# zyddnys/manga-image-translator

Hardware: AMD Instinct MI355X
Metric: pages/sec end-to-end (detect+OCR+inpaint), 2048x1456 (higher is better)
Workload: dtype f32

## Files before the change

### include/mit_hip.h

```cpp
#ifndef MIT_HIP_H
#define MIT_HIP_H

#include <stdint.h>

#ifdef __cplusplus
extern "C" {
#endif

#define MIT_ABI_VERSION 23
#define MIT_MAX_TAPS 64

enum MitAct {
    MIT_ACT_NONE = 0,
    MIT_ACT_RELU = 1,
    MIT_ACT_LEAKY = 2,
    MIT_ACT_SILU = 3,
    MIT_ACT_SIGMOID = 4,
    MIT_ACT_GELU = 5
};
#define MIT_ACT_POST_FIRST 0x100

enum MitPad {
    MIT_PAD_ZERO = 0,
    MIT_PAD_REFLECT = 1
};

typedef struct MitTensorMap {
    float *base;
    int64_t zs1, zs0, bs, ys, xs;
    int64_t nhi;
    int32_t nsplit;
    int32_t _pad;
} MitTensorMap;

typedef struct MitConvGemm {
    const float *a;
    int64_t a_zs1, a_zs0, a_bs, a_ys, a_xs;
    int32_t NB, Hi, Wi, Cin;
    int32_t Ho, Wo, sy, sx;
    int32_t ntaps, pad_mode;
    int8_t tap_dy[MIT_MAX_TAPS];
    int8_t tap_dx[MIT_MAX_TAPS];
    int32_t tap_off[MIT_MAX_TAPS];
    const float *w;
    int64_t w_zs1, w_zs0, ldw;
    int32_t Kw, Nw;
    int32_t N;
    int32_t Z, zdiv;
    MitTensorMap c, pre, post;
    const float *scale, *bias;
    int32_t act;
    float act_alpha;
    const uint16_t *w_split;
    int64_t ws_zs0;
    const int32_t *lut_rows;
    const float *lut1, *lut2;
    int64_t lut_ld;
    int32_t nprod;
    int32_t live_img0;
    const int32_t *live_blocks;
    const int32_t *live_start;
    const float *wino_m;
// ... 1 lines not shown
    int32_t wino_n, wino_th, wino_tw;
    int32_t _pad_wino;
} MitConvGemm;

const char *mit_last_error(void);
int mit_abi_version(void);
const char *mit_source_digest(void);

int mit_device_count(int *count);
int mit_device_name(int device, char *buf, int buflen);

int mit_conv_gemm(const MitConvGemm *desc, void *stream);
int mit_conv_gemm_cfg(const MitConvGemm *desc, int cfg, void *stream);
const char *mit_conv_gemm_config_name(int cfg);
int mit_conv_gemm_plan(const MitConvGemm *desc, int cfg, int32_t *tile, int32_t *nb_run);
const char *mit_conv_gemm_config_kernel(int cfg);

int mit_gemm_split_pack(const float *w_dev, int64_t w_zs, int nz, int Kw, int64_t ldw, uint16_t *out_dev, void *stream);
int mit_gemm_mode_set(int mode);
int mit_gemm_mode_get(void);
int64_t mit_gemm_split_min_tiles(int64_t n);

typedef struct MitPGemm {
    const uint16_t *a_planes;
    int64_t a_zs;
    int64_t lda;
    const uint16_t *w_planes;
    int64_t w_zs;
    int64_t ldw;
    int32_t M, N, K, Z;
    float *c;
    int64_t ldc, c_zs;
    const float *pre;
    int64_t ld_pre, pre_zs;
    const float *post;
    int64_t ld_post, post_zs;
    uint16_t *c_planes;
    int64_t ld_cp, cp_zs;
    const float *scale, *bias;
    int32_t act;
    float act_alpha;
    int32_t nprod;
    int32_t tile;
} MitPGemm;
int mit_pgemm(const MitPGemm *desc, void *stream);
const char *mit_pgemm_tile_name(int tile);
int mit_pgemm_supported(const MitPGemm *desc);
int mit_split_planes(const float *x_dev, int64_t ldx, int R, int K, uint16_t *planes_dev, int64_t ld, void *stream);
int mit_join_planes(const uint16_t *planes_dev, int64_t ld, int R, int K, float *x_dev, int64_t ldx, void *stream);

int mit_conv_small_cout(const float *in_dev, int64_t in_pixstride, int64_t in_planestride, const float *w4_dev, const float *w_pairs_dev, const float *bias_dev, float *out_dev,
                        int64_t out_pixstride, int B, int H, int W, int Cin, int Cout, int k, int pad_mode, int act,
                        float act_alpha, const uint8_t *live_cells, void *stream);

int64_t mit_lama_tail_need_work(int B, int H, int W);
int mit_lama_tail_need(const uint8_t *mask_dev, int B, int H, int W, uint8_t *cells_dev, int32_t *list0_dev, int32_t *start0_dev, int32_t *list1_dev,
                       int32_t *start1_dev, int32_t *list2_dev, int32_t *start2_dev, uint8_t *work_dev, void *stream);

int mit_convnext_mlp_supported(int C);
int mit_convnext_mlp(const float *x_dev, int64_t ldx, int M, int C, const uint16_t *w1_planes_dev, const float *b1_dev,
                     const uint16_t *w2perm_planes_dev, int64_t ldn2, const float *scale2_dev, const float *bias2_dev,
                     const float *post_dev, int64_t ldp, float *out_dev, int64_t ldo, void *stream);

int mit_wino43_input(const float *x_dev, int64_t x_bs, int64_t x_ys, int64_t x_xs, float *v_dev, int B, int H, int W, int C,
                     int pad_mode, void *stream);
int mit_wino43_output(const float *m_dev, float *y_dev, int64_t y_bs, int64_t y_ys, int64_t y_xs, const float *post_dev,
                      int64_t p_bs, int64_t p_ys, int64_t p_xs, const float *scale_dev, const float *bias_dev, int B, int H,
                      int W, int N, int act, float alpha, void *stream);

typedef struct MitProfStat {
    int64_t launches;
    double ms, exec_flops, alg_flops;
} MitProfStat;
int mit_prof_enable(int on);
int mit_prof_tag_next(double alg_flops);
int mit_prof_read(MitProfStat *stats, int max_cfgs, int *n_cfgs);
int mit_prof_dump(const char *path);
typedef struct MitProfKernelStat {
    char name[48];
    int64_t launches;
    double ms, alg_bytes, alg_flops;
} MitProfKernelStat;
int mit_prof_kernels_read(MitProfKernelStat *stats, int max_stats, int *n_stats);

int mit_resize_u8(const uint8_t *src_dev, int B, int H, int W, int C, uint8_t *dst_dev, int dh, int dw, int mode, const int *yidx_dev,
                  const uint16_t *ycoef_dev, const int *xidx_dev, const uint16_t *xcoef_dev, void *stream);
int mit_resample_pil_u8(const uint8_t *src_dev, int B, int H, int W, int C, uint8_t *dst_dev, int n_out, int axis, const int *bounds_dev,
                        const int *coef_dev, int ksize, void *stream);
int mit_bilateral_u8c3(const uint8_t *src_dev, uint8_t *dst_dev, int B, int H, int W, int radius, int ntaps, const int *tap_ofs_dev,
                       const float *tap_w_dev, const float *color_w_dev, void *stream);
int mit_select_u8(const uint8_t *mask_dev, int thr, const uint8_t *a_dev, const uint8_t *b_dev, uint8_t *out_dev, int64_t npix, int C,
                  void *stream);

typedef struct MitRefineWindow {
    int x1, y1, x2, y2;
} MitRefineWindow;
typedef struct MitRefineCand {
    int kind;
    int lo, hi;
    int invert;
} MitRefineCand;
int64_t mit_ctd_refine_workspace_bytes(const MitRefineWindow *windows, int n);
int mit_ctd_refine_hist(const uint8_t *page_dev, const uint8_t *pred_dev, int H, int W, const MitRefineWindow *windows, int n, int *hist_host,
                        void *workspace_dev, int64_t workspace_bytes, void *stream);
int mit_ctd_refine_scores(const uint8_t *page_dev, const uint8_t *pred_dev, int H, int W, const MitRefineWindow *windows, int n,
                          const MitRefineCand *cands_host, uint64_t *sums_host, void *workspace_dev, int64_t workspace_bytes, void *stream);
// ... 285 lines not shown
```

### manga_image_translator_amd/ctd.py

```python
from __future__ import annotations

import ctypes as C
import math
from typing import Dict, Optional, Tuple

import numpy as np
import torch

from . import lib as _lib
from . import ops
from .ops import ACT_LEAKY, ACT_NONE, ACT_RELU, ACT_SIGMOID, ACT_SILU, bn_params

INPUT_SIZE = 1024


def _fused_yolo_conv(sd, p, k, s, device):
    w = sd[p + ".conv.weight"].to(torch.float32)
    bw, bb, rm, rv = (sd[p + ".bn." + n].to(torch.float32) for n in ("weight", "bias", "running_mean", "running_var"))
    eps = 1e-3
    scale = bw.div(torch.sqrt(eps + rv))
    fw = (w.reshape(w.shape[0], -1) * scale[:, None]).reshape(w.shape)
    fb = bb - bw.mul(rm).div(torch.sqrt(rv + eps))
    return ops.Conv2d(fw, fb, stride=s, padding=(2 if k == 6 else k // 2), act=ACT_SILU, device=device)


def _head_conv(sd, p, k, device):
    return ops.Conv2d(sd[p + ".conv.weight"], None, padding=k // 2, bn=bn_params(sd, p + ".bn"), act=ACT_LEAKY, alpha=0.1,
                      device=device)


class _C3:

    def __init__(self, sd, p, c1, c2, n, mk, shortcut=True):
        self.c_ = c2 // 2
        self.c2 = c2
        self.cv1, self.cv2, self.cv3 = mk(p + ".cv1", 1), mk(p + ".cv2", 1), mk(p + ".cv3", 1)
        self.m = [(mk(f"{p}.m.{j}.cv1", 1), mk(f"{p}.m.{j}.cv2", 3)) for j in range(n)]
        self.shortcut = shortcut

    def __call__(self, eng, x, out, tag):
        B, H, W, _ = x.shape
        cat = eng._buf(f"{tag}.cat", B, H, W, 2 * self.c_)
        y = cat[..., :self.c_]
        self.cv2(x, out=cat[..., self.c_:])
        self.cv1(x, out=y)
        t = eng._buf(f"{tag}.t", B, H, W, self.c_)
        for a, b in self.m:
            a(y, out=t)
            b(t, out=y, post=y if self.shortcut else None)
        return self.cv3(cat, out=out)


class CtdEngine(ops.Engine):

    def __init__(self, yolo_sd: Dict[str, torch.Tensor], seg_sd: Dict[str, torch.Tensor], det_sd: Dict[str, torch.Tensor],
                 device="cuda"):
        super().__init__(device)
        dev = self.device
        ymk = lambda k_s: (lambda p, k: _fused_yolo_conv(yolo_sd, p, k, k_s, dev))
        y1 = lambda p, k: _fused_yolo_conv(yolo_sd, p, k, 1, dev)
        self.y0 = _fused_yolo_conv(yolo_sd, "model.0", 6, 2, dev)
        self.y1 = _fused_yolo_conv(yolo_sd, "model.1", 3, 2, dev)
        self.y2 = _C3(yolo_sd, "model.2", 64, 64, 1, y1)
        self.y3 = _fused_yolo_conv(yolo_sd, "model.3", 3, 2, dev)
        self.y4 = _C3(yolo_sd, "model.4", 128, 128, 2, y1)
        self.y5 = _fused_yolo_conv(yolo_sd, "model.5", 3, 2, dev)
        self.y6 = _C3(yolo_sd, "model.6", 256, 256, 3, y1)
        self.y7 = _fused_yolo_conv(yolo_sd, "model.7", 3, 2, dev)
        self.y8 = _C3(yolo_sd, "model.8", 512, 512, 1, y1)
        self.y9a = y1("model.9.cv1", 1)
        self.y9b = y1("model.9.cv2", 1)

        def up_c3(sd, p, cin, mid, cout):
            hk = lambda q, k: _head_conv(sd, q, k, dev)
            c3 = _C3(sd, p + ".conv.0", cin, mid, 1, hk)
            up = ops.ConvTranspose2d(sd[p + ".conv.1.weight"], None, stride=2, padding=1, bn=bn_params(sd, p + ".conv.2"),
                                     act=ACT_RELU, device=dev)
            return c3, up

        s = seg_sd
        self.down1 = _C3(s, "down_conv1.conv", 512, 512, 1, lambda q, k: _head_conv(s, q, k, dev))
        self.up0 = up_c3(s, "upconv0", 512, 512, 256)
        self.up2 = up_c3(s, "upconv2", 768, 512, 256)
        self.up3 = up_c3(s, "upconv3", 512, 512, 256)
        self.up4 = up_c3(s, "upconv4", 384, 256, 128)
        self.up5 = up_c3(s, "upconv5", 192, 128, 64)
        self.up6 = ops.ConvTranspose2d(s["upconv6.0.weight"], None, stride=2, padding=1, act=ACT_SIGMOID, device=dev)
        d = det_sd
        self.d_up3 = up_c3(d, "upconv3", 512, 512, 256)
        self.d_up4 = up_c3(d, "upconv4", 384, 256, 128)
        self.d_conv = ops.Conv2d(d["conv.0.weight"], d["conv.0.bias"], bn=bn_params(d, "conv.1"), act=ACT_RELU, device=dev)

        def branch(p, first_bias):
            c0 = ops.Conv2d(d[p + ".0.weight"], d[p + ".0.bias"] if first_bias else None, padding=1, bn=bn_params(d, p + ".1"),
                            act=ACT_RELU, device=dev)
            t1 = ops.ConvTranspose2d(d[p + ".3.weight"], d[p + ".3.bias"], stride=2, bn=bn_params(d, p + ".4"), act=ACT_RELU,
                                     device=dev)
            t2 = ops.ConvTranspose2d(d[p + ".6.weight"], d[p + ".6.bias"], stride=2, act=ACT_SIGMOID, device=dev)
            return c0, t1, t2

        self.br_binarize = branch("binarize", True)
        self.br_thresh = branch("thresh", False)
        self._prep_tabs: Dict[Tuple, dict] = {}

    @staticmethod
    def letterbox_geometry(H: int, W: int, S: int = INPUT_SIZE):
        r = min(S / H, S / W)
        nw, nh = int(round(W * r)), int(round(H * r))
        return nh, nw, S - nw, S - nh

    def _resize_tables(self, H, W, nh, nw):
# ... 45 lines not shown
        if (nh, nw) == (H, W):
            mode, tb = 0, None
        elif H == 2 * nh and W == 2 * nw:
            mode, tb = 1, None
        else:
            mode, tb = 2, self._resize_tables(H, W, nh, nw)
        _lib.check(lib.mit_ctd_prep(pages_u8.data_ptr(), B, H, W, nh, nw, S, mode,
                                    tb["yi"].data_ptr() if tb else None, tb["yc"].data_ptr() if tb else None,
                                    tb["xi"].data_ptr() if tb else None, tb["xc"].data_ptr() if tb else None,
                                    x.data_ptr(), st), "mit_ctd_prep")
        if taps is not None:
            taps["input"] = x.clone()
        a0 = self._buf("y0", B, 512, 512, 32)
        self.y0(x, out=a0)
        cat160 = self._buf("cat160", B, 256, 256, 192)
        f160 = cat160[..., :64]
        self.y1(a0, out=f160)
        a2 = self._buf("y2", B, 256, 256, 64)
        self.y2(self, f160, a2, "y2")
        cat80 = self._buf("cat80", B, 128, 128, 384)
        f80 = cat80[..., :128]
        self.y3(a2, out=f80)
        a4 = self._buf("y4", B, 128, 128, 128)
        self.y4(self, f80, a4, "y4")
        cat40 = self._buf("cat40", B, 64, 64, 512)
        f40 = cat40[..., :256]
        self.y5(a4, out=f40)
        a6 = self._buf("y6", B, 64, 64, 256)
        self.y6(self, f40, a6, "y6")
        cat20 = self._buf("cat20", B, 32, 32, 768)
        f20 = cat20[..., :512]
        self.y7(a6, out=f20)
        a8 = self._buf("y8", B, 32, 32, 512)
        self.y8(self, f20, a8, "y8")
        sp = self._buf("sppf", B, 32, 32, 1024)
        self.y9a(a8, out=sp[..., :256])
        for j in range(3):
            src, dst = sp[..., 256 * j:256 * (j + 1)], sp[..., 256 * (j + 1):256 * (j + 2)]
            _lib.check(lib.mit_maxpool_nhwc(src.data_ptr(), 1024, dst.data_ptr(), 1024, B, 32, 32, 256, 5, st), "mit_maxpool_nhwc")
        f3 = self._buf("f3", B, 32, 32, 512)
        self.y9b(sp, out=f3)
        if taps is not None:
            taps.update(f160=f160.clone(), f80=f80.clone(), f40=f40.clone(), f20=f20.clone(), f3=f3.clone())
        p16 = self._buf("p16", B, 16, 16, 512)
        _lib.check(lib.mit_avgpool2_nhwc(f3.data_ptr(), 512, p16.data_ptr(), 512, B, 16, 16, 512, st), "mit_avgpool2_nhwc")
        d10 = self._buf("d10", B, 16, 16, 512)
        self.down1(self, p16, d10, "down1")
        self._up(self.up0, d10, cat20[..., 512:], "up0")
        self._up(self.up2, cat20, cat40[..., 256:], "up2")
        self._up(self.up3, cat40, cat80[..., 128:], "up3")
        self._up(self.up4, cat80, cat160[..., 64:], "up4")
        u320 = self._buf("u320", B, 512, 512, 64)
        self._up(self.up5, cat160, u320, "up5")
        mask = self._buf("mask", B, S, S, 1)
        self.up6(u320, out=mask)
        dcat80 = self._buf("dcat80", B, 128, 128, 384)
        _lib.check(lib.mit_copy_channels(f80.data_ptr(), 384, dcat80.data_ptr(), 384, B * 128 * 128, 128, st), "mit_copy_channels")
        self._up(self.d_up3, cat40, dcat80[..., 128:], "dup3")
        dx = self._buf("dx", B, 256, 256, 128)
        self._up(self.d_up4, dcat80, dx, "dup4")
        dc = self._buf("dc", B, 256, 256, 64)
        self.d_conv(dx, out=dc)
        lines = self._buf("lines", B, 2, S, S)
        for plane, (c0, t1, t2) in ((0, self.br_binarize), (1, self.br_thresh)):
            b0 = self._buf("db0", B, 256, 256, 16)
            c0(dc, out=b0)
            b1 = self._buf("db1", B, 512, 512, 16)
            t1(b0, out=b1)
            t2(b1, out=lines[:, plane].unsqueeze(-1))
        mask_u8 = self._buf("mask_u8", B, S, S, dtype=torch.uint8)
        _lib.check(lib.mit_map_to_u8(mask.data_ptr(), mask_u8.data_ptr(), B * S * S, 0, 0.0, st), "mit_map_to_u8")
        if taps is not None:
            taps["mask_f32"] = mask.clone()
        self.last_mask_f32 = mask[..., 0]
        return mask_u8[:, :S - dh, :S - dw], lines[:, :, :S - dh, :S - dw], (dw, dh)

    def shrink_bitmap(self, lines: torch.Tensor, thr: float = 0.3) -> torch.Tensor:
        shrink = lines[:, 0].contiguous()
        out = torch.empty(shrink.shape, dtype=torch.uint8, device=self.device)
        _lib.check(_lib.load().mit_map_to_u8(shrink.data_ptr(), out.data_ptr(), shrink.numel(), 1, thr,
                                             C.c_void_p(ops.current_stream())), "mit_map_to_u8")
        return out

    @staticmethod
    def flops_per_page() -> float:
        def conv(cin, cout, k, hw):
            return 2.0 * cin * cout * k * k * hw

        def c3(c1, c2, n, hw):
            c_ = c2 // 2
            return conv(c1, c_, 1, hw) * 2 + conv(2 * c_, c2, 1, hw) + n * (conv(c_, c_, 1, hw) + conv(c_, c_, 3, hw))

        f = conv(3, 32, 6, 512 ** 2) + conv(32, 64, 3, 256 ** 2) + c3(64, 64, 1, 256 ** 2) + conv(64, 128, 3, 128 ** 2)
        f += c3(128, 128, 2, 128 ** 2) + conv(128, 256, 3, 64 ** 2) + c3(256, 256, 3, 64 ** 2) + conv(256, 512, 3, 32 ** 2)
        f += c3(512, 512, 1, 32 ** 2) + conv(512, 256, 1, 32 ** 2) + conv(1024, 512, 1, 32 ** 2)

        def up(cin, mid, cout, hw):
            return c3(cin, mid, 1, hw) + conv(mid, cout, 4, hw)

        f += c3(512, 512, 1, 16 ** 2) + up(512, 512, 256, 16 ** 2) + up(768, 512, 256, 32 ** 2) + up(512, 512, 256, 64 ** 2)
        f += up(384, 256, 128, 128 ** 2) + up(192, 128, 64, 256 ** 2) + conv(64, 1, 4, 512 ** 2)
        f += up(512, 512, 256, 64 ** 2) + up(384, 256, 128, 128 ** 2) + conv(128, 64, 1, 256 ** 2)
        f += 2 * (conv(64, 16, 3, 256 ** 2) + conv(16, 16, 2, 256 ** 2) + conv(16, 1, 2, 512 ** 2))
        return f
```

### manga_image_translator_amd/lib.py

```python
from __future__ import annotations

import ctypes as C
from pathlib import Path

MIT_MAX_TAPS = 64
MIT_ABI_VERSION = 23

ACT_NONE, ACT_RELU, ACT_LEAKY, ACT_SILU, ACT_SIGMOID, ACT_GELU = range(6)
ACT_POST_FIRST = 0x100
PAD_ZERO, PAD_REFLECT = 0, 1


class MitTensorMap(C.Structure):
    _fields_ = [
        ("base", C.c_void_p),
        ("zs1", C.c_int64),
        ("zs0", C.c_int64),
        ("bs", C.c_int64),
        ("ys", C.c_int64),
        ("xs", C.c_int64),
        ("nhi", C.c_int64),
        ("nsplit", C.c_int32),
        ("_pad", C.c_int32),
    ]


class MitConvGemm(C.Structure):
    _fields_ = [
        ("a", C.c_void_p),
        ("a_zs1", C.c_int64),
        ("a_zs0", C.c_int64),
        ("a_bs", C.c_int64),
        ("a_ys", C.c_int64),
        ("a_xs", C.c_int64),
        ("NB", C.c_int32),
        ("Hi", C.c_int32),
        ("Wi", C.c_int32),
        ("Cin", C.c_int32),
        ("Ho", C.c_int32),
        ("Wo", C.c_int32),
        ("sy", C.c_int32),
        ("sx", C.c_int32),
        ("ntaps", C.c_int32),
        ("pad_mode", C.c_int32),
        ("tap_dy", C.c_int8 * MIT_MAX_TAPS),
        ("tap_dx", C.c_int8 * MIT_MAX_TAPS),
        ("tap_off", C.c_int32 * MIT_MAX_TAPS),
        ("w", C.c_void_p),
        ("w_zs1", C.c_int64),
        ("w_zs0", C.c_int64),
        ("ldw", C.c_int64),
        ("Kw", C.c_int32),
        ("Nw", C.c_int32),
        ("N", C.c_int32),
        ("Z", C.c_int32),
        ("zdiv", C.c_int32),
        ("c", MitTensorMap),
        ("pre", MitTensorMap),
        ("post", MitTensorMap),
# ... 85 lines not shown
    _fields_ = [("name", C.c_char * 48), ("launches", C.c_int64), ("ms", C.c_double), ("alg_bytes", C.c_double),
                ("alg_flops", C.c_double)]


class MitWarpLine(C.Structure):
    _fields_ = [("minv", C.c_double * 9), ("page", C.c_int32), ("x1", C.c_int32), ("y1", C.c_int32), ("cw", C.c_int32),
                ("ch", C.c_int32), ("dw", C.c_int32), ("dh", C.c_int32), ("vertical", C.c_int32), ("out_row", C.c_int32),
                ("_pad", C.c_int32)]


class MitCrfCrop(C.Structure):
    _fields_ = [("x", C.c_int32), ("y", C.c_int32), ("w", C.c_int32), ("h", C.c_int32)]


class MitDilateJob(C.Structure):
    _fields_ = [("sx", C.c_int32), ("sy", C.c_int32), ("sw", C.c_int32), ("sh", C.c_int32), ("dx", C.c_int32), ("dy", C.c_int32),
                ("dw", C.c_int32), ("dh", C.c_int32), ("k", C.c_int32), ("spitch", C.c_int32), ("src_off", C.c_int64)]


class MitMaskRun(C.Structure):
    _fields_ = [("y", C.c_int32), ("x0", C.c_int32), ("x1", C.c_int32), ("comp", C.c_int32)]


class MitRefineWindow(C.Structure):
    _fields_ = [("x1", C.c_int32), ("y1", C.c_int32), ("x2", C.c_int32), ("y2", C.c_int32)]


class MitRefineCand(C.Structure):
    _fields_ = [("kind", C.c_int32), ("lo", C.c_int32), ("hi", C.c_int32), ("invert", C.c_int32)]


class MitRaggedSeg(C.Structure):
    _fields_ = [("pixel_start", C.c_int64), ("group_start", C.c_int64), ("B", C.c_int32), ("H", C.c_int32), ("W", C.c_int32),
                ("_pad", C.c_int32)]


SYMBOLS = {
    "mit_last_error": (C.c_char_p, []),
    "mit_abi_version": (C.c_int, []),
    "mit_source_digest": (C.c_char_p, []),
    "mit_device_count": (C.c_int, [C.POINTER(C.c_int)]),
    "mit_device_name": (C.c_int, [C.c_int, C.c_char_p, C.c_int]),
    "mit_conv_gemm": (C.c_int, [C.POINTER(MitConvGemm), C.c_void_p]),
    "mit_conv_gemm_cfg": (C.c_int, [C.POINTER(MitConvGemm), C.c_int, C.c_void_p]),
    "mit_conv_gemm_config_name": (C.c_char_p, [C.c_int]),
    "mit_conv_gemm_plan": (C.c_int, [C.POINTER(MitConvGemm), C.c_int, C.POINTER(C.c_int32), C.POINTER(C.c_int32)]),
    "mit_conv_gemm_config_kernel": (C.c_char_p, [C.c_int]),
    "mit_gemm_split_pack": (C.c_int, [C.c_void_p, C.c_int64, C.c_int, C.c_int, C.c_int64, C.c_void_p, C.c_void_p]),
    "mit_gemm_mode_set": (C.c_int, [C.c_int]),
    "mit_gemm_mode_get": (C.c_int, []),
    "mit_gemm_split_min_tiles": (C.c_int64, [C.c_int64]),
    "mit_conv_small_cout": (C.c_int, [C.c_void_p, C.c_int64, C.c_int64, C.c_void_p, C.c_void_p, C.c_void_p, C.c_void_p, C.c_int64, C.c_int, C.c_int,
                                      C.c_int, C.c_int, C.c_int, C.c_int, C.c_int, C.c_int, C.c_float, C.c_void_p, C.c_void_p]),
    "mit_lama_tail_need_work": (C.c_int64, [C.c_int, C.c_int, C.c_int]),
    "mit_lama_tail_need": (C.c_int, [C.c_void_p, C.c_int, C.c_int, C.c_int] + [C.c_void_p] * 9),
    "mit_convnext_mlp_supported": (C.c_int, [C.c_int]),
    "mit_convnext_mlp": (C.c_int, [C.c_void_p, C.c_int64, C.c_int, C.c_int, C.c_void_p, C.c_void_p, C.c_void_p, C.c_int64, C.c_void_p, C.c_void_p,
                                   C.c_void_p, C.c_int64, C.c_void_p, C.c_int64, C.c_void_p]),
    "mit_prof_enable": (C.c_int, [C.c_int]),
    "mit_prof_tag_next": (C.c_int, [C.c_double]),
    "mit_prof_read": (C.c_int, [C.POINTER(MitProfStat), C.c_int, C.POINTER(C.c_int)]),
    "mit_prof_dump": (C.c_int, [C.c_char_p]),
    "mit_prof_kernels_read": (C.c_int, [C.POINTER(MitProfKernelStat), C.c_int, C.POINTER(C.c_int)]),
    "mit_wino43_input": (C.c_int, [C.c_void_p, C.c_int64, C.c_int64, C.c_int64, C.c_void_p, C.c_int, C.c_int, C.c_int, C.c_int, C.c_int,
                                   C.c_void_p]),
    "mit_wino43_output": (C.c_int, [C.c_void_p, C.c_void_p, C.c_int64, C.c_int64, C.c_int64, C.c_void_p, C.c_int64, C.c_int64, C.c_int64,
                                    C.c_void_p, C.c_void_p, C.c_int, C.c_int, C.c_int, C.c_int, C.c_int, C.c_float, C.c_void_p]),
    "mit_ocr_warp_lines": (C.c_int, [C.c_void_p, C.c_int, C.c_int, C.c_void_p, C.c_int, C.c_void_p, C.c_int, C.c_int,
                                     C.c_void_p]),
    "mit_fft_cols": (C.c_int, [C.c_void_p, C.c_int64, C.c_int64, C.c_int64, C.c_void_p, C.c_int64, C.c_int64, C.c_int64,
                               C.c_void_p, C.c_int, C.c_int, C.c_int64, C.c_int, C.c_float, C.c_void_p]),
    "mit_rfft_rows_supported": (C.c_int, [C.c_int]),
    "mit_rfft_rows": (C.c_int, [C.c_void_p, C.c_int64, C.c_int64, C.c_int64, C.c_void_p, C.c_int64, C.c_int64, C.c_int64, C.c_int64,
                                C.c_void_p, C.c_int, C.c_int, C.c_int, C.c_int, C.c_float, C.c_void_p]),
    "mit_irfft_rows": (C.c_int, [C.c_void_p, C.c_int64, C.c_int64, C.c_int64, C.c_int64, C.c_void_p, C.c_int64, C.c_int64, C.c_int64,
                                 C.c_void_p, C.c_int64, C.c_int64, C.c_int64, C.c_void_p, C.c_int, C.c_int, C.c_int, C.c_int,
                                 C.c_float, C.c_void_p]),
    "mit_bilateral_u8c3": (C.c_int, [C.c_void_p, C.c_void_p, C.c_int, C.c_int, C.c_int, C.c_int, C.c_int, C.c_void_p, C.c_void_p,
                                     C.c_void_p, C.c_void_p]),
    "mit_mask_dilate_jobs": (C.c_int, [C.c_void_p, C.c_void_p, C.c_int, C.c_void_p, C.c_int, C.c_int, C.c_int, C.c_void_p, C.c_void_p]),
    "mit_binarize_u8": (C.c_int, [C.c_void_p, C.c_int64, C.c_void_p]),
    "mit_densecrf_workspace_bytes": (C.c_int64, [C.c_void_p, C.c_int]),
    "mit_densecrf_refine": (C.c_int, [C.c_void_p, C.c_int, C.c_int, C.c_void_p, C.c_int, C.c_void_p, C.c_void_p, C.c_void_p, C.c_float,
                                      C.c_float, C.c_float, C.c_float, C.c_float, C.c_int, C.c_void_p, C.c_void_p, C.c_int64, C.c_void_p]),
    "mit_ctd_refine_workspace_bytes": (C.c_int64, [C.c_void_p, C.c_int]),
    "mit_ctd_refine_hist": (C.c_int, [C.c_void_p, C.c_void_p, C.c_int, C.c_int, C.c_void_p, C.c_int, C.c_void_p, C.c_void_p, C.c_int64,
                                      C.c_void_p]),
    "mit_ctd_refine_scores": (C.c_int, [C.c_void_p, C.c_void_p, C.c_int, C.c_int, C.c_void_p, C.c_int, C.c_void_p, C.c_void_p, C.c_void_p,
                                        C.c_int64, C.c_void_p]),
    "mit_ctd_refine_merge": (C.c_int, [C.c_void_p, C.c_void_p, C.c_int, C.c_int, C.c_void_p, C.c_int, C.c_void_p, C.c_void_p, C.c_void_p,
                                       C.c_int64, C.c_void_p]),
    "mit_lama_prep": (C.c_int, [C.c_void_p, C.c_void_p, C.c_void_p, C.c_int, C.c_int, C.c_int, C.c_void_p]),
    "mit_lama_prep_padded": (C.c_int, [C.c_void_p, C.c_void_p, C.c_void_p, C.c_int, C.c_int, C.c_int, C.c_int, C.c_int, C.c_void_p]),
    "mit_lama_mpe_index": (C.c_int, [C.c_void_p, C.c_int, C.c_int, C.c_int, C.c_void_p, C.c_void_p, C.c_void_p,
                                     C.c_int, C.c_void_p, C.c_void_p, C.c_void_p, C.c_int, C.c_void_p, C.c_void_p,
                                     C.c_void_p, C.c_void_p]),
    "mit_lama_mpe_add": (C.c_int, [C.c_void_p, C.c_void_p, C.c_void_p, C.c_void_p, C.c_void_p, C.c_void_p,
                                   C.c_void_p, C.c_void_p, C.c_float, C.c_float, C.c_int, C.c_int, C.c_int,
                                   C.c_void_p]),
    "mit_lama_mpe_rows": (C.c_int, [C.c_void_p, C.c_void_p, C.c_void_p, C.c_void_p, C.c_void_p, C.c_void_p, C.c_int, C.c_int, C.c_int, C.c_void_p]),
    "mit_ctd_prep": (C.c_int, [C.c_void_p, C.c_int, C.c_int, C.c_int, C.c_int, C.c_int, C.c_int, C.c_int, C.c_void_p,
                               C.c_void_p, C.c_void_p, C.c_void_p, C.c_void_p, C.c_void_p]),
    "mit_maxpool_nhwc": (C.c_int, [C.c_void_p, C.c_int64, C.c_void_p, C.c_int64, C.c_int, C.c_int, C.c_int, C.c_int,
                                   C.c_int, C.c_void_p]),
    "mit_maxpool2d_nhwc": (C.c_int, [C.c_void_p, C.c_void_p, C.c_int, C.c_int, C.c_int, C.c_int, C.c_int, C.c_int, C.c_int,
                                     C.c_void_p]),
# ... 164 lines not shown
```

### manga_image_translator_amd/ops.py

```python
from __future__ import annotations

import ctypes as C
import math
import os
import weakref
from dataclasses import dataclass, field
from typing import Dict, List, Optional, Sequence, Tuple

import torch

from . import lib as _lib
from .lib import (ACT_GELU, ACT_LEAKY, ACT_NONE, ACT_POST_FIRST, ACT_RELU, ACT_SIGMOID, ACT_SILU, MIT_MAX_TAPS, PAD_REFLECT,
                  PAD_ZERO, MitConvGemm, MitPGemm, MitTensorMap)

__all__ = [
    "ACT_NONE", "ACT_RELU", "ACT_LEAKY", "ACT_SILU", "ACT_SIGMOID", "ACT_GELU", "ACT_POST_FIRST", "PAD_ZERO", "PAD_REFLECT",
    "Conv2d", "ConvSmallCout", "split_mode", "ensure_split", "set_split_mode", "gemm_mode", "ConvTranspose2d", "UpsampleConv2d", "fold_bn", "conv_gemm_desc", "launch_conv_gemm", "current_stream",
]


def current_stream() -> int:
    return torch.cuda.current_stream().cuda_stream


# ... 318 lines not shown
    register_split(out)
    return out, Kp, Np


@dataclass
class _Packed:
    w: torch.Tensor
    Kp: int
    Np: int
    taps: List[Tuple[int, int, int]]


class Conv2d:

    def __init__(self, weight: torch.Tensor, bias: Optional[torch.Tensor] = None, *, stride=1, padding=0,
                 pad_mode: int = PAD_ZERO, bn=None, act: int = ACT_NONE, alpha: float = 0.0, device="cuda",
                 out_scale: Optional[torch.Tensor] = None, dilation: int = 1):
        Cout, Cin, kh, kw = weight.shape
        self.Cout, self.Cin_raw = Cout, Cin
        self.Cin = _round_up(Cin, 4)
        self.kh, self.kw = kh, kw
        self.sy, self.sx = (stride, stride) if isinstance(stride, int) else stride
        self.py, self.px = (padding, padding) if isinstance(padding, int) else padding
        self.d = int(dilation)
        if self.d < 1:
            raise ValueError(f"Conv2d: dilation must be >= 1 (got {dilation})")
        self.pad_mode = pad_mode
        self.act, self.alpha = act, alpha
        w = weight.detach().to(torch.float32)
        if self.Cin != Cin:
            w = torch.cat([w, torch.zeros(Cout, self.Cin - Cin, kh, kw)], dim=1)
        w_kn = w.permute(2, 3, 1, 0).reshape(kh * kw * self.Cin, Cout)
        self.w, self.Kp, self.Np = pack_weight_kn(w_kn, device)
        self.taps = [(ky * self.d - self.py, kx * self.d - self.px, 0) for ky in range(kh) for kx in range(kw)]
        scale = bias_t = None
        if bn is not None:
            scale, bias_t = fold_bn(*bn, conv_bias=bias)
        elif bias is not None:
            bias_t = bias.detach().to(torch.float32)
        if out_scale is not None:
            os_ = out_scale.detach().to(torch.float32).reshape(-1)
            scale = os_ if scale is None else scale * os_
            if bias_t is not None:
                bias_t = bias_t * os_
        self.scale = None if scale is None else scale.to(device).contiguous()
        self.bias = None if bias_t is None else bias_t.to(device).contiguous()

    def out_hw(self, H: int, W: int) -> Tuple[int, int]:
        d = self.d
        return ((H + 2 * self.py - d * (self.kh - 1) - 1) // self.sy + 1, (W + 2 * self.px - d * (self.kw - 1) - 1) // self.sx + 1)

    def desc(self, x: torch.Tensor, out: torch.Tensor, pre: Optional[torch.Tensor] = None,
             post: Optional[torch.Tensor] = None, nprod: int = 0, wino_pre: Optional[torch.Tensor] = None,
             live: Optional[Tuple[torch.Tensor, torch.Tensor]] = None) -> MitConvGemm:
        _check_nhwc(x, "Conv2d input")
        if nprod:
            ensure_split(self.w)
        _check_nhwc(out, "Conv2d output")
        B, H, W, Cx = x.shape
        if Cx != self.Cin:
            raise ValueError(f"Conv2d: input has {Cx} channels, layer expects {self.Cin}")
        Ho, Wo = self.out_hw(H, W)
        if tuple(out.shape) != (B, Ho, Wo, self.Cout):
            raise ValueError(f"Conv2d: output shape {tuple(out.shape)} != {(B, Ho, Wo, self.Cout)}")
        for t, nm in ((pre, "pre"), (post, "post")):
            if t is not None and tuple(t.shape) != tuple(out.shape):
                raise ValueError(f"Conv2d: {nm} shape {tuple(t.shape)} != output {tuple(out.shape)}")
        return conv_gemm_desc(
            a=x, NB=B, Hi=H, Wi=W, Cin=self.Cin, a_strides=(x.stride(0), x.stride(1), x.stride(2)), Ho=Ho, Wo=Wo,
            sy=self.sy, sx=self.sx, taps=self.taps, pad_mode=self.pad_mode, w=self.w, ldw=self.Np, Kw=self.Kp,
            Nw=self.Np, N=self.Cout, c=tensor_map(out), pre=tensor_map(pre), post=tensor_map(post),
            scale=self.scale, bias=self.bias, act=self.act, alpha=self.alpha, nprod=nprod, wino_pre=wino_pre,
            live=full_block_list(B, Ho, Wo, x.device) if wino_pre is not None and live is None else live)

    def __call__(self, x: torch.Tensor, out: Optional[torch.Tensor] = None, pre: Optional[torch.Tensor] = None,
                 post: Optional[torch.Tensor] = None, cfg: int = -1, nprod: int = 0, wino_pre: Optional[torch.Tensor] = None) -> torch.Tensor:
        if out is None:
            Ho, Wo = self.out_hw(x.shape[1], x.shape[2])
            out = torch.empty(x.shape[0], Ho, Wo, self.Cout, dtype=torch.float32, device=x.device)
        launch_conv_gemm(self.desc(x, out, pre, post, nprod, wino_pre), cfg)
        return out


class WinogradConv3x3:

    G = ((1 / 4, 0, 0), (-1 / 6, -1 / 6, -1 / 6), (-1 / 6, 1 / 6, -1 / 6), (1 / 24, 1 / 12, 1 / 6), (1 / 24, -1 / 12, 1 / 6), (0, 0, 1))

    def __init__(self, weight: torch.Tensor, bias: Optional[torch.Tensor] = None, *, pad_mode: int = PAD_ZERO, bn=None,
                 act: int = ACT_NONE, alpha: float = 0.0, device="cuda"):
        Cout, Cin, kh, kw = weight.shape
        if (kh, kw) != (3, 3) or Cin % 4 or Cout % 2:
            raise ValueError(f"WinogradConv3x3: 3x3 kernels with Cin % 4 == 0 and even Cout only (got {tuple(weight.shape)})")
        if act not in (ACT_NONE, ACT_RELU, ACT_LEAKY):
            raise ValueError("WinogradConv3x3: activation must be none / relu / leaky")
        self.Cin, self.Cout, self.pad_mode, self.act, self.alpha = Cin, Cout, pad_mode, act, alpha
        G = torch.tensor(self.G, dtype=torch.float64)
        U = torch.einsum("ia,ocab,jb->ijco", G, weight.detach().to(torch.float64), G).reshape(36, Cin, Cout)
        self.Kp, self.Np = _round_up(Cin, 16), _round_up(Cout, 4)
        u = torch.zeros(36, self.Kp, self.Np, dtype=torch.float32)
        u[:, :Cin, :Cout] = U.to(torch.float32)
        self.u = u.to(device).contiguous()
        register_split(self.u)
        scale = bias_t = None
        if bn is not None:
            scale, bias_t = fold_bn(*bn, conv_bias=bias)
        elif bias is not None:
            bias_t = bias.detach().to(torch.float32)
        self.scale = None if scale is None else scale.to(device).contiguous()
        self.bias = None if bias_t is None else bias_t.to(device).contiguous()

    @staticmethod
    def tiles(B: int, H: int, W: int) -> int:
        return B * ((H + 3) // 4) * ((W + 3) // 4)

    def transform_input(self, x: torch.Tensor, v: torch.Tensor) -> torch.Tensor:
        _check_nhwc(x, "WinogradConv3x3 input")
        B, H, W, Cx = x.shape
        T = self.tiles(B, H, W)
        if tuple(v.shape) != (36, T, Cx) or not v.is_contiguous():
            raise ValueError(f"WinogradConv3x3: V must be contiguous [36, {T}, {Cx}] (got {tuple(v.shape)})")
        _lib.check(_lib.load().mit_wino43_input(x.data_ptr(), x.stride(0), x.stride(1), x.stride(2), v.data_ptr(), B, H, W, Cx,
                                                self.pad_mode, C.c_void_p(current_stream())), "mit_wino43_input")
        return v

    def gemm_desc(self, v: torch.Tensor, m: torch.Tensor) -> MitConvGemm:
        _, T, Cv = v.shape
        if Cv < self.Cin or tuple(m.shape) != (36, T, self.Cout) or not m.is_contiguous():
            raise ValueError(f"WinogradConv3x3: bad V / M shapes {tuple(v.shape)} / {tuple(m.shape)}")
        cm = MitTensorMap()
        cm.base, cm.zs1, cm.zs0, cm.bs, cm.ys, cm.xs = m.data_ptr(), 0, T * self.Cout, 0, 0, self.Cout
        return conv_gemm_desc(a=v, NB=1, Hi=1, Wi=T, Cin=self.Cin, a_strides=(0, 0, Cv), Ho=1, Wo=T, sy=1, sx=1, taps=[(0, 0, 0)],
                              pad_mode=PAD_ZERO, w=self.u, ldw=self.Np, Kw=self.Kp, Nw=self.Np, N=self.Cout, c=cm, Z=36,
                              zdiv=1 << 30, a_zs=(0, T * Cv), w_zs=(0, self.Kp * self.Np))
# ... 101 lines not shown
        _check_nhwc(out, "UpsampleConv2d output")
        B, H, W, Cx = x.shape
        if Cx != self.Cin or tuple(out.shape) != (B, 2 * H, 2 * W, self.Cout):
            raise ValueError(f"UpsampleConv2d: bad shapes {tuple(x.shape)} -> {tuple(out.shape)}")
        ds = []
        for a, b, pk in self.sub:
            ov = out[:, a::2, b::2]
            ds.append(conv_gemm_desc(
                a=x, NB=B, Hi=H, Wi=W, Cin=self.Cin, a_strides=(x.stride(0), x.stride(1), x.stride(2)), Ho=H, Wo=W, sy=1, sx=1,
                taps=pk.taps, pad_mode=PAD_ZERO, w=pk.w, ldw=pk.Np, Kw=pk.Kp, Nw=pk.Np, N=self.Cout, c=tensor_map(ov),
                bias=self.bias, act=self.act, alpha=self.alpha))
        return ds

    def __call__(self, x: torch.Tensor, out: Optional[torch.Tensor] = None, cfg: int = -1) -> torch.Tensor:
        if out is None:
            out = torch.empty(x.shape[0], 2 * x.shape[1], 2 * x.shape[2], self.Cout, dtype=torch.float32, device=x.device)
        for d in self.descs(x, out):
            launch_conv_gemm(d, cfg)
        return out


class ConvTranspose2d:

    def __init__(self, weight: torch.Tensor, bias: Optional[torch.Tensor] = None, *, stride=2, padding=0,
                 output_padding=0, bn=None, act: int = ACT_NONE, alpha: float = 0.0, device="cuda"):
        Cin, Cout, kh, kw = weight.shape
        if Cin % 4:
            raise ValueError("ConvTranspose2d: Cin must be a multiple of 4")
        self.Cin, self.Cout, self.k, self.s, self.p, self.op = Cin, Cout, (kh, kw), stride, padding, output_padding
        self.act, self.alpha = act, alpha
        w = weight.detach().to(torch.float32)
        self.sub: List[Tuple[int, int, _Packed]] = []
        s, p = stride, padding
        for py in range(s):
            kys = [ky for ky in range(kh) if (py + p - ky) % s == 0]
            for px in range(s):
                kxs = [kx for kx in range(kw) if (px + p - kx) % s == 0]
                taps, blocks = [], []
                for ky in kys:
                    for kx in kxs:
                        taps.append(((py + p - ky) // s, (px + p - kx) // s, 0))
                        blocks.append(w[:, :, ky, kx])
                if not taps:
                    raise ValueError("ConvTranspose2d: empty parity class (kernel smaller than stride)")
                wk, Kp, Np = pack_weight_kn(torch.cat(blocks, dim=0), device)
                self.sub.append((py, px, _Packed(wk, Kp, Np, taps)))
        scale = bias_t = None
        if bn is not None:
            scale, bias_t = fold_bn(*bn, conv_bias=bias)
        elif bias is not None:
            bias_t = bias.detach().to(torch.float32)
        self.scale = None if scale is None else scale.to(device).contiguous()
        self.bias = None if bias_t is None else bias_t.to(device).contiguous()

    def out_hw(self, H: int, W: int) -> Tuple[int, int]:
        return ((H - 1) * self.s - 2 * self.p + self.k[0] + self.op, (W - 1) * self.s - 2 * self.p + self.k[1] + self.op)

    def descs(self, x: torch.Tensor, out: torch.Tensor, planes: int = 0, parity_major: bool = False, nprod: int = 0,
              live: Optional[Tuple[torch.Tensor, torch.Tensor]] = None) -> List[MitConvGemm]:
        split = nhi = 0
        if planes:
            if out.dim() != 5 or out.shape[0] != planes or out.shape[4] * planes != self.Cout or not out.is_contiguous():
                raise ValueError(f"ConvTranspose2d: planar output must be contiguous [{planes}, B, Ho, Wo, {self.Cout // planes}]")
            split, nhi = out.shape[4], out.stride(0)
            out = out[0].as_strided((out.shape[1], out.shape[2], out.shape[3], self.Cout), (out.stride(1), out.stride(2), out.stride(3), 1))
        _check_nhwc(x, "ConvTranspose2d input")
        _check_nhwc(out, "ConvTranspose2d output")
        B, H, W, Cx = x.shape
        if Cx != self.Cin:
            raise ValueError(f"ConvTranspose2d: input has {Cx} channels, layer expects {self.Cin}")
        Ho, Wo = self.out_hw(H, W)
        if tuple(out.shape) != (B, Ho, Wo, self.Cout):
            raise ValueError(f"ConvTranspose2d: output shape {tuple(out.shape)} != {(B, Ho, Wo, self.Cout)}")
        if parity_major and not (planes and self.s == 2 and Ho % 2 == 0 and Wo % 2 == 0):
            raise ValueError("ConvTranspose2d: the parity-major layout is for planar output of a stride-2 layer with even output size")
        ds = []
        for py, px, pk in self.sub:
            ov = out[:, py::self.s, px::self.s]
            if live is not None and (ov.shape[1] * self.s != Ho or ov.shape[2] * self.s != Wo):
                raise ValueError("ConvTranspose2d: a live-block list needs an output size that is a multiple of the stride")
            if ov.shape[1] == 0 or ov.shape[2] == 0:
                continue
            if nprod:
                ensure_split(pk.w)
            if parity_major:
                pc, h2, w2 = self.Cout // planes, Ho // 2, Wo // 2
                ov = out.as_strided((B, h2, w2, self.Cout), (Ho * Wo * pc, w2 * pc, pc, 1),
                                    out.storage_offset() + (py * 2 + px) * h2 * w2 * pc)
            ds.append(conv_gemm_desc(
                a=x, NB=B, Hi=H, Wi=W, Cin=self.Cin, a_strides=(x.stride(0), x.stride(1), x.stride(2)),
                Ho=ov.shape[1], Wo=ov.shape[2], sy=1, sx=1, taps=pk.taps, pad_mode=PAD_ZERO, w=pk.w, ldw=pk.Np,
                Kw=pk.Kp, Nw=pk.Np, N=self.Cout, c=tensor_map(ov, nsplit=split, nhi=nhi), scale=self.scale, bias=self.bias, act=self.act,
                alpha=self.alpha, nprod=nprod, live=live))
        return ds

    def __call__(self, x: torch.Tensor, out: Optional[torch.Tensor] = None, cfg: int = -1, planes: int = 0, parity_major: bool = False,
                 nprod: int = 0, live: Optional[Tuple[torch.Tensor, torch.Tensor]] = None) -> torch.Tensor:
        if out is None:
            Ho, Wo = self.out_hw(x.shape[1], x.shape[2])
            out = (torch.empty(planes, x.shape[0], Ho, Wo, self.Cout // planes, dtype=torch.float32, device=x.device) if planes else
                   torch.empty(x.shape[0], Ho, Wo, self.Cout, dtype=torch.float32, device=x.device))
        for d in self.descs(x, out, planes, parity_major, nprod, live):
            launch_conv_gemm(d, cfg)
        return out
```

Before: 46.55.

## Add single-pass Cout=1 transposed-conv kernel and crop detector heads to valid extent

```diff
diff --git a/include/mit_hip.h b/include/mit_hip.h
--- a/include/mit_hip.h
+++ b/include/mit_hip.h
@@ -7,7 +7,7 @@
 extern "C" {
 #endif
 
-#define MIT_ABI_VERSION 23
+#define MIT_ABI_VERSION 24
 #define MIT_MAX_TAPS 64
 
 enum MitAct {
@@ -115,6 +115,12 @@
 int mit_conv_small_cout(const float *in_dev, int64_t in_pixstride, int64_t in_planestride, const float *w4_dev, const float *w_pairs_dev, const float *bias_dev, float *out_dev,
                         int64_t out_pixstride, int B, int H, int W, int Cin, int Cout, int k, int pad_mode, int act,
                         float act_alpha, const uint8_t *live_cells, void *stream);
+
+#define MIT_CONVT_COUT1_STRIP_K4 16
+#define MIT_CONVT_COUT1_STRIP_K2 64
+int mit_convt_cout1(const float *x_dev, int64_t x_bs, int64_t x_ys, int64_t x_xs, int B, int Hi, int Wi, int Cin, const float *w_dev, int k,
+                    int stride, int pad, const float *scale_dev, const float *bias_dev, int act, float act_alpha, float *out_dev,
+                    int64_t out_bs, int64_t out_ys, int64_t out_xs, int out_h, int out_w, void *stream);
 
 int64_t mit_lama_tail_need_work(int B, int H, int W);
 int mit_lama_tail_need(const uint8_t *mask_dev, int B, int H, int W, uint8_t *cells_dev, int32_t *list0_dev, int32_t *start0_dev, int32_t *list1_dev,
diff --git a/manga_image_translator_amd/csrc/convt_cout1.hip b/manga_image_translator_amd/csrc/convt_cout1.hip
--- /dev/null
+++ b/manga_image_translator_amd/csrc/convt_cout1.hip
@@ -0,0 +1,175 @@
+#include "conv_gemm_kernels.h"
+
+namespace {
+
+template <int K>
+struct Geo {
+    static constexpr int LPR = K == 4 ? 16 : 4;
+    static constexpr int CPW = 64 / LPR;
+    static constexpr int STRIP = 4 * CPW;
+    static constexpr int ROWS = K == 4 ? 16 : 8;
+    static constexpr int OFF = K == 4 ? 1 : 0;
+};
+
+struct Args {
+    const float *x;
+    int64_t x_bs, x_ys, x_xs;
+    int Hi, Wi;
+    const float *w, *scale, *bias;
+    int act;
+    float act_alpha;
+    float *out;
+    int64_t o_bs, o_ys, o_xs;
+    int out_h, out_w, ncy, ncx;
+};
+
+__device__ __forceinline__ float fma4(const f32x4 v, const float w0, const float w1, const float w2, const float w3, float acc) {
+    acc = __builtin_fmaf(v.x, w0, acc);
+    acc = __builtin_fmaf(v.y, w1, acc);
+    acc = __builtin_fmaf(v.z, w2, acc);
+    acc = __builtin_fmaf(v.w, w3, acc);
+    return acc;
+}
+
+template <int K>
+__global__ __launch_bounds__(256) void convt_cout1_kernel(const Args p) {
+    using G = Geo<K>;
+    constexpr int LPR = G::LPR, KK = K * K;
+    const int lane = threadIdx.x & 63, wave = threadIdx.x >> 6;
+    const int sub = lane % LPR, slot = lane / LPR;
+    const int cx = (blockIdx.x * 4 + wave) * G::CPW + slot;
+    const int j = cx - G::OFF;
+    const int cy0 = blockIdx.y * G::ROWS;
+    const bool cok = cx < p.ncx;
+    const float *xb = p.x + (int64_t)blockIdx.z * p.x_bs + sub * 4;
+
+    float wr[4][KK];
+#pragma unroll
+    for (int c = 0; c < 4; ++c)
+#pragma unroll
+        for (int t = 0; t < KK; t += 4) {
+            const f32x4 w4 = *reinterpret_cast<const f32x4 *>(p.w + (sub * 4 + c) * KK + t);
+            wr[c][t] = w4.x, wr[c][t + 1] = w4.y, wr[c][t + 2] = w4.z, wr[c][t + 3] = w4.w;
+        }
+
+    auto in_img = [&](const int iy, const int ix) -> bool { return cok && iy >= 0 && iy < p.Hi && ix >= 0 && ix < p.Wi; };
+    auto ld = [&](const int iy, const int ix) -> f32x4 {
+        const int y = iy < 0 ? 0 : (iy >= p.Hi ? p.Hi - 1 : iy), x = ix < 0 ? 0 : (ix >= p.Wi ? p.Wi - 1 : ix);
+        return *reinterpret_cast<const f32x4 *>(xb + (int64_t)y * p.x_ys + (int64_t)x * p.x_xs);
+    };
+    const int X = 2 * j + G::OFF + (sub & 1);
+    const bool xok = cok && sub < 4 && X >= 0 && X < p.out_w;
+    float *ob = p.out + (int64_t)blockIdx.z * p.o_bs + (int64_t)X * p.o_xs;
+    const float scale = p.scale ? p.scale[0] : 1.f, bias = p.bias ? p.bias[0] : 0.f;
+
+    const int i0 = cy0 - G::OFF;
+    const f32x4 zero4 = {0.f, 0.f, 0.f, 0.f};
+    f32x4 t0 = zero4, t1 = zero4, n0, n1 = zero4;
+    bool nok0, nok1 = false;
+    if (K == 4) {
+        t0 = in_img(i0, j) ? ld(i0, j) : zero4, t1 = in_img(i0, j + 1) ? ld(i0, j + 1) : zero4;
+        n0 = ld(i0 + 1, j), n1 = ld(i0 + 1, j + 1);
+        nok0 = in_img(i0 + 1, j), nok1 = in_img(i0 + 1, j + 1);
+    } else {
+        n0 = ld(i0, j);
+        nok0 = in_img(i0, j);
+    }
+#pragma unroll 1
+    for (int r = 0; r < G::ROWS; ++r) {
+        const int cy = cy0 + r;
+        if (cy >= p.ncy) break;
+        const int i = cy - G::OFF;
+        const f32x4 b0 = nok0 ? n0 : zero4, b1 = nok1 ? n1 : zero4;
+        const int iyn = i + (K == 4 ? 2 : 1);
+        const bool more = r + 1 < G::ROWS && cy + 1 < p.ncy;
+        n0 = ld(iyn, j);
+        nok0 = more && in_img(iyn, j);
+        if (K == 4) {
+            n1 = ld(iyn, j + 1);
+            nok1 = more && in_img(iyn, j + 1);
+        }
+
+        float acc[2][2];
+#pragma unroll
+        for (int a = 0; a < 2; ++a)
+#pragma unroll
+            for (int b = 0; b < 2; ++b) {
+                float s = 0.f;
+                if (K == 4) {
+                    const int k11 = a * 4 + b, k10 = a * 4 + b + 2, k01 = (a + 2) * 4 + b, k00 = (a + 2) * 4 + b + 2;
+                    s = fma4(b1, wr[0][k11], wr[1][k11], wr[2][k11], wr[3][k11], s);
+                    s = fma4(b0, wr[0][k10], wr[1][k10], wr[2][k10], wr[3][k10], s);
+                    s = fma4(t1, wr[0][k01], wr[1][k01], wr[2][k01], wr[3][k01], s);
+                    s = fma4(t0, wr[0][k00], wr[1][k00], wr[2][k00], wr[3][k00], s);
+                } else {
+                    const int k0 = a * 2 + b;
+                    s = fma4(b0, wr[0][k0], wr[1][k0], wr[2][k0], wr[3][k0], s);
+                }
+#pragma unroll
+                for (int o = LPR / 2; o > 0; o >>= 1) s += __shfl_xor(s, o);
+                acc[a][b] = s;
+            }
+        const int a = sub >> 1;
+        const int Y = 2 * i + G::OFF + a;
+        if (xok && Y >= 0 && Y < p.out_h) {
+            float v = (sub & 2) ? ((sub & 1) ? acc[1][1] : acc[1][0]) : ((sub & 1) ? acc[0][1] : acc[0][0]);
+            v = v * scale + bias;
+            switch (p.act) {
+                case MIT_ACT_RELU: v = mitcg::apply_act<MIT_ACT_RELU>(v, p.act_alpha); break;
+                case MIT_ACT_LEAKY: v = mitcg::apply_act<MIT_ACT_LEAKY>(v, p.act_alpha); break;
+                case MIT_ACT_SILU: v = mitcg::apply_act<MIT_ACT_SILU>(v, p.act_alpha); break;
+                case MIT_ACT_SIGMOID: v = mitcg::apply_act<MIT_ACT_SIGMOID>(v, p.act_alpha); break;
+                case MIT_ACT_GELU: v = mitcg::apply_act<MIT_ACT_GELU>(v, p.act_alpha); break;
+                default: break;
+            }
+            ob[(int64_t)Y * p.o_ys] = v;
+        }
+        if (K == 4) t0 = b0, t1 = b1;
+    }
+}
+
+template <int K>
+void launch(const Args &a, int B, hipStream_t st) {
+    using G = Geo<K>;
+    dim3 grid((a.ncx + G::STRIP - 1) / G::STRIP, (a.ncy + G::ROWS - 1) / G::ROWS, B);
+    hipLaunchKernelGGL(convt_cout1_kernel<K>, grid, dim3(256), 0, st, a);
+}
+
+}
+
+static_assert(Geo<4>::STRIP == MIT_CONVT_COUT1_STRIP_K4 && Geo<2>::STRIP == MIT_CONVT_COUT1_STRIP_K2, "strip widths of mit_hip.h");
+
+extern "C" int mit_convt_cout1(const float *x_dev, int64_t x_bs, int64_t x_ys, int64_t x_xs, int B, int Hi, int Wi, int Cin, const float *w_dev, int k,
+                               int stride, int pad, const float *scale_dev, const float *bias_dev, int act, float act_alpha, float *out_dev,
+                               int64_t out_bs, int64_t out_ys, int64_t out_xs, int out_h, int out_w, void *stream) {
+    if (!x_dev || !w_dev || !out_dev) return mit_set_error("mit_convt_cout1: null pointer");
+    if (!(stride == 2 && ((k == 4 && pad == 1 && Cin == 64) || (k == 2 && pad == 0 && Cin == 16))))
+        return mit_set_error("mit_convt_cout1: only k4 s2 p1 at Cin = 64 and k2 s2 p0 at Cin = 16 (got k%d s%d p%d, Cin = %d)", k, stride, pad, Cin);
+    if (B <= 0 || B > 65535 || Hi <= 0 || Wi <= 0) return mit_set_error("mit_convt_cout1: need 0 < B < 65536 and a non-empty input");
+    if (out_h <= 0 || out_w <= 0 || out_h > 2 * (int64_t)Hi || out_w > 2 * (int64_t)Wi)
+        return mit_set_error("mit_convt_cout1: extent %d x %d is not inside the layer's output %lld x %lld", out_h, out_w, 2LL * Hi, 2LL * Wi);
+    if ((reinterpret_cast<uintptr_t>(x_dev) & 15) || (reinterpret_cast<uintptr_t>(w_dev) & 15) || (x_bs & 3) || (x_ys & 3) || (x_xs & 3))
+        return mit_set_error("mit_convt_cout1: x and w must be 16-byte aligned, the input strides multiples of 4 floats");
+    if (act != MIT_ACT_NONE && act != MIT_ACT_RELU && act != MIT_ACT_LEAKY && act != MIT_ACT_SILU && act != MIT_ACT_SIGMOID && act != MIT_ACT_GELU)
+        return mit_set_error("mit_convt_cout1: unknown activation %d", act);
+    Args a;
+    a.x = x_dev, a.x_bs = x_bs, a.x_ys = x_ys, a.x_xs = x_xs, a.Hi = Hi, a.Wi = Wi;
+    a.w = w_dev, a.scale = scale_dev, a.bias = bias_dev, a.act = act, a.act_alpha = act_alpha;
+    a.out = out_dev, a.o_bs = out_bs, a.o_ys = out_ys, a.o_xs = out_xs, a.out_h = out_h, a.out_w = out_w;
+    int rows_in, cols_in;
+    if (k == 4) {
+        a.ncy = (out_h >> 1) + 1, a.ncx = (out_w >> 1) + 1;
+        rows_in = a.ncy < Hi ? a.ncy : Hi, cols_in = a.ncx < Wi ? a.ncx : Wi;
+    } else {
+        a.ncy = rows_in = (out_h + 1) >> 1, a.ncx = cols_in = (out_w + 1) >> 1;
+    }
+    if ((a.ncy + 7) / 8 > 65535) return mit_set_error("mit_convt_cout1: extent exceeds the grid");
+    hipStream_t st = (hipStream_t)stream;
+    MitProbeScope probe("convt_cout1_kernel", st, 4.0 * B * ((double)rows_in * cols_in * Cin + (double)out_h * out_w));
+    if (k == 4)
+        launch<4>(a, B, st);
+    else
+        launch<2>(a, B, st);
+    MIT_CHECK_LAUNCH("mit_convt_cout1");
+    return 0;
+}
diff --git a/manga_image_translator_amd/ctd.py b/manga_image_translator_amd/ctd.py
--- a/manga_image_translator_amd/ctd.py
+++ b/manga_image_translator_amd/ctd.py
@@ -27,6 +27,14 @@
 def _head_conv(sd, p, k, device):
     return ops.Conv2d(sd[p + ".conv.weight"], None, padding=k // 2, bn=bn_params(sd, p + ".bn"), act=ACT_LEAKY, alpha=0.1,
                       device=device)
+
+
+def head_extents(hv: int, wv: int, S: int = INPUT_SIZE) -> Tuple[Tuple[int, int], Tuple[int, int], Tuple[int, int]]:
+    half = lambda n: (n + 1) // 2
+    b1 = (half(hv), half(wv))
+    b0 = (half(b1[0]), half(b1[1]))
+    u = (min(S // 2, b1[0] + 1), min(S // 2, b1[1] + 1))
+    return u, b1, b0
 
 
 class _C3:
@@ -54,9 +62,10 @@
 class CtdEngine(ops.Engine):
 
     def __init__(self, yolo_sd: Dict[str, torch.Tensor], seg_sd: Dict[str, torch.Tensor], det_sd: Dict[str, torch.Tensor],
-                 device="cuda"):
+                 device="cuda", fused_heads: bool = True):
         super().__init__(device)
         dev = self.device
+        self.fused_heads = bool(fused_heads)
         ymk = lambda k_s: (lambda p, k: _fused_yolo_conv(yolo_sd, p, k, k_s, dev))
         y1 = lambda p, k: _fused_yolo_conv(yolo_sd, p, k, 1, dev)
         self.y0 = _fused_yolo_conv(yolo_sd, "model.0", 6, 2, dev)
@@ -208,8 +217,12 @@
         self._up(self.up4, cat80, cat160[..., 64:], "up4")
         u320 = self._buf("u320", B, 512, 512, 64)
         self._up(self.up5, cat160, u320, "up5")
+        hv, wv = S - dh, S - dw
         mask = self._buf("mask", B, S, S, 1)
-        self.up6(u320, out=mask)
+        if self.fused_heads:
+            self.up6.single_pass(u320, mask, hv, wv)
+        else:
+            self.up6(u320, out=mask)
         dcat80 = self._buf("dcat80", B, 128, 128, 384)
         _lib.check(lib.mit_copy_channels(f80.data_ptr(), 384, dcat80.data_ptr(), 384, B * 128 * 128, 128, st), "mit_copy_channels")
         self._up(self.d_up3, cat40, dcat80[..., 128:], "dup3")
@@ -220,16 +233,23 @@
         lines = self._buf("lines", B, 2, S, S)
         for plane, (c0, t1, t2) in ((0, self.br_binarize), (1, self.br_thresh)):
             b0 = self._buf("db0", B, 256, 256, 16)
-            c0(dc, out=b0)
             b1 = self._buf("db1", B, 512, 512, 16)
-            t1(b0, out=b1)
-            t2(b1, out=lines[:, plane].unsqueeze(-1))
+            if self.fused_heads:
+                _, _, (h0, w0) = head_extents(hv, wv, S)
+                b0v = b0[:, :h0, :w0]
+                c0(dc, out=b0v, out_hw=(h0, w0))
+                t1(b0v, out=b1[:, :2 * h0, :2 * w0])
+                t2.single_pass(b1, lines[:, plane].unsqueeze(-1), hv, wv)
+            else:
+                c0(dc, out=b0)
+                t1(b0, out=b1)
+                t2(b1, out=lines[:, plane].unsqueeze(-1))
         mask_u8 = self._buf("mask_u8", B, S, S, dtype=torch.uint8)
         _lib.check(lib.mit_map_to_u8(mask.data_ptr(), mask_u8.data_ptr(), B * S * S, 0, 0.0, st), "mit_map_to_u8")
         if taps is not None:
             taps["mask_f32"] = mask.clone()
-        self.last_mask_f32 = mask[..., 0]
-        return mask_u8[:, :S - dh, :S - dw], lines[:, :, :S - dh, :S - dw], (dw, dh)
+        self.last_mask_f32 = mask[:, :hv, :wv, 0]
+        return mask_u8[:, :hv, :wv], lines[:, :, :hv, :wv], (dw, dh)
 
     def shrink_bitmap(self, lines: torch.Tensor, thr: float = 0.3) -> torch.Tensor:
         shrink = lines[:, 0].contiguous()
diff --git a/manga_image_translator_amd/lib.py b/manga_image_translator_amd/lib.py
--- a/manga_image_translator_amd/lib.py
+++ b/manga_image_translator_amd/lib.py
@@ -4,7 +4,7 @@
 from pathlib import Path
 
 MIT_MAX_TAPS = 64
-MIT_ABI_VERSION = 23
+MIT_ABI_VERSION = 24
 
 ACT_NONE, ACT_RELU, ACT_LEAKY, ACT_SILU, ACT_SIGMOID, ACT_GELU = range(6)
 ACT_POST_FIRST = 0x100
@@ -196,6 +196,8 @@
     "mit_gemm_split_min_tiles": (C.c_int64, [C.c_int64]),
     "mit_conv_small_cout": (C.c_int, [C.c_void_p, C.c_int64, C.c_int64, C.c_void_p, C.c_void_p, C.c_void_p, C.c_void_p, C.c_int64, C.c_int, C.c_int,
                                       C.c_int, C.c_int, C.c_int, C.c_int, C.c_int, C.c_int, C.c_float, C.c_void_p, C.c_void_p]),
+    "mit_convt_cout1": (C.c_int, [C.c_void_p, C.c_int64, C.c_int64, C.c_int64, C.c_int, C.c_int, C.c_int, C.c_int, C.c_void_p, C.c_int, C.c_int, C.c_int,
+                                  C.c_void_p, C.c_void_p, C.c_int, C.c_float, C.c_void_p, C.c_int64, C.c_int64, C.c_int64, C.c_int, C.c_int, C.c_void_p]),
     "mit_lama_tail_need_work": (C.c_int64, [C.c_int, C.c_int, C.c_int]),
     "mit_lama_tail_need": (C.c_int, [C.c_void_p, C.c_int, C.c_int, C.c_int] + [C.c_void_p] * 9),
     "mit_convnext_mlp_supported": (C.c_int, [C.c_int]),
diff --git a/manga_image_translator_amd/ops.py b/manga_image_translator_amd/ops.py
--- a/manga_image_translator_amd/ops.py
+++ b/manga_image_translator_amd/ops.py
@@ -394,7 +394,7 @@
 
     def desc(self, x: torch.Tensor, out: torch.Tensor, pre: Optional[torch.Tensor] = None,
              post: Optional[torch.Tensor] = None, nprod: int = 0, wino_pre: Optional[torch.Tensor] = None,
-             live: Optional[Tuple[torch.Tensor, torch.Tensor]] = None) -> MitConvGemm:
+             live: Optional[Tuple[torch.Tensor, torch.Tensor]] = None, out_hw: Optional[Tuple[int, int]] = None) -> MitConvGemm:
         _check_nhwc(x, "Conv2d input")
         if nprod:
             ensure_split(self.w)
@@ -403,6 +403,10 @@
         if Cx != self.Cin:
             raise ValueError(f"Conv2d: input has {Cx} channels, layer expects {self.Cin}")
         Ho, Wo = self.out_hw(H, W)
+        if out_hw is not None:
+            if not (0 < out_hw[0] <= Ho and 0 < out_hw[1] <= Wo):
+                raise ValueError(f"Conv2d: out_hw {tuple(out_hw)} is not inside the output {(Ho, Wo)}")
+            Ho, Wo = out_hw
         if tuple(out.shape) != (B, Ho, Wo, self.Cout):
             raise ValueError(f"Conv2d: output shape {tuple(out.shape)} != {(B, Ho, Wo, self.Cout)}")
         for t, nm in ((pre, "pre"), (post, "post")):
@@ -416,11 +420,12 @@
             live=full_block_list(B, Ho, Wo, x.device) if wino_pre is not None and live is None else live)
 
     def __call__(self, x: torch.Tensor, out: Optional[torch.Tensor] = None, pre: Optional[torch.Tensor] = None,
-                 post: Optional[torch.Tensor] = None, cfg: int = -1, nprod: int = 0, wino_pre: Optional[torch.Tensor] = None) -> torch.Tensor:
+                 post: Optional[torch.Tensor] = None, cfg: int = -1, nprod: int = 0, wino_pre: Optional[torch.Tensor] = None,
+                 out_hw: Optional[Tuple[int, int]] = None) -> torch.Tensor:
         if out is None:
-            Ho, Wo = self.out_hw(x.shape[1], x.shape[2])
+            Ho, Wo = self.out_hw(x.shape[1], x.shape[2]) if out_hw is None else out_hw
             out = torch.empty(x.shape[0], Ho, Wo, self.Cout, dtype=torch.float32, device=x.device)
-        launch_conv_gemm(self.desc(x, out, pre, post, nprod, wino_pre), cfg)
+        launch_conv_gemm(self.desc(x, out, pre, post, nprod, wino_pre, out_hw=out_hw), cfg)
         return out
 
 
@@ -628,9 +633,27 @@
             bias_t = bias.detach().to(torch.float32)
         self.scale = None if scale is None else scale.to(device).contiguous()
         self.bias = None if bias_t is None else bias_t.to(device).contiguous()
+        self.one_pass = Cout == 1 and stride == 2 and output_padding == 0 and (kh, kw, padding, Cin) in ((4, 4, 1, 64), (2, 2, 0, 16))
+        self.w_raw = w.to(device).contiguous() if self.one_pass else None
 
     def out_hw(self, H: int, W: int) -> Tuple[int, int]:
         return ((H - 1) * self.s - 2 * self.p + self.k[0] + self.op, (W - 1) * self.s - 2 * self.p + self.k[1] + self.op)
+
+    def single_pass(self, x: torch.Tensor, out: torch.Tensor, out_h: Optional[int] = None, out_w: Optional[int] = None) -> torch.Tensor:
+        if not self.one_pass:
+            raise ValueError("ConvTranspose2d.single_pass: only Cout = 1 layers of k4 s2 p1 (Cin 64) or k2 s2 (Cin 16)")
+        _check_nhwc(x, "ConvTranspose2d input")
+        B, H, W, Cx = x.shape
+        if Cx != self.Cin or tuple(out.shape) != (B, 2 * H, 2 * W, 1):
+            raise ValueError(f"ConvTranspose2d.single_pass: bad shapes {tuple(x.shape)} -> {tuple(out.shape)}")
+        if out.dtype != torch.float32 or out.device != x.device:
+            raise ValueError("ConvTranspose2d.single_pass: fp32 output on the input's device required")
+        out_h, out_w = 2 * H if out_h is None else out_h, 2 * W if out_w is None else out_w
+        _lib.check(_lib.load().mit_convt_cout1(x.data_ptr(), x.stride(0), x.stride(1), x.stride(2), B, H, W, self.Cin, self.w_raw.data_ptr(),
+                                               self.k[0], self.s, self.p, _ptr(self.scale), _ptr(self.bias), self.act, self.alpha,
+                                               out.data_ptr(), out.stride(0), out.stride(1), out.stride(2), out_h, out_w,
+                                               C.c_void_p(current_stream())), "mit_convt_cout1")
+        return out
 
     def descs(self, x: torch.Tensor, out: torch.Tensor, planes: int = 0, parity_major: bool = False, nprod: int = 0,
               live: Optional[Tuple[torch.Tensor, torch.Tensor]] = None) -> List[MitConvGemm]:
```

After: 47.05, median of 6. +1.1%, better.
